# Jackz915/PackPPI

Measured on AMD Instinct MI355X. Metric: sampled residues/sec at 100 diffusion steps, higher is better.
Workload: dtype f32 (dense layers as split-f16: two f16 per operand, three f16 MFMAs per product, fp32 accumulate); 1 GPU; data/T1124_lig.pdb (L=739, 738 true residues), 1 complex per GPU; diffusion_steps=100, proximal=False, residues_per_gpu=738, residues_rank0=738, residues_total=738, mode=ode

## Files before the change

include/packppi_hip.h:

```cpp
#ifndef PACKPPI_HIP_H
#define PACKPPI_HIP_H

#include <stddef.h>
#include <stdint.h>

#ifdef __cplusplus
extern "C" {
#endif

typedef enum pp_status {
    PP_OK = 0,
    PP_ERR_INVALID = 1,
    PP_ERR_HIP = 2,
    PP_ERR_UNSUPPORTED = 3,
    PP_ERR_NO_DEVICE = 4
} pp_status;

typedef struct pp_plan pp_plan;
typedef struct pp_ctx pp_ctx;

#define PP_N_WEIGHTS 1439172u
#define PP_HIDDEN 128
#define PP_TOP_K 32
#define PP_MODE_ODE 0
// ... 216 lines not shown
#define PP_REFINE_MOVED 22
#define PP_REFINE_PCAP 16
#define PP_REFINE_MAX_SWEEPS 256
#define PP_REFINE_MAX_STEPS 16
#define PP_REFINE_MAX_BANDS 8
pp_status pp_chi_refine(pp_ctx *ctx, const float *chi0 , const uint8_t *fixed ,
                        const int8_t *place , const float *param ,
                        const float *ext , const float *radius ,
                        const uint8_t *acls , const uint8_t *aa_sep ,
                        const int32_t *link , const uint8_t *obst_polar , float delta,
                        int max_steps, int bands, float band, float cut, float hb_allow, float hb_weak, float hb_weak2, float hb_good2,
                        float reach, int max_sweeps, float *chi_out , int8_t *steps ,
                        float *xyz_out , float *hxyz_out ,
                        uint8_t *hmask_out , uint8_t *link_prev , int32_t *e ,
                        int32_t *trace , int32_t *sweeps ,
                        int32_t *converged , float *cand_xyz, float *cand_hxyz, uint8_t *cand_hmask,
                        int32_t *cand_mask, int32_t *energy , void *stream);

pp_status pp_time_kernel(pp_ctx *ctx, int which, int iters, float *avg_ms, void *stream);

pp_status pp_profile_kernel(pp_ctx *ctx, int which);
pp_status pp_profile_read(pp_ctx *ctx, float *total_ms, int *launches);

int pp_edge_variant(void);

int pp_has_range_check(void);
pp_status pp_range_check(unsigned long long *events, int reset);
pp_status pp_range_check_parts(unsigned long long *edge_events, unsigned long long *node_events, int reset);

pp_status pp_ctx_saturated(pp_ctx *ctx, int *flags, void *stream);

pp_status pp_ctx_live_rows(pp_ctx *ctx, int32_t *rows, int *count, void *stream);

#ifdef PP_DIAG
pp_status pp_debug_edge(pp_ctx *ctx, int layer, void *stream);
pp_status pp_debug_nm(pp_ctx *ctx, int layer, void *stream);
pp_status pp_debug_set_hE(pp_ctx *ctx, const float *src, size_t n);
pp_status pp_debug_buffer(pp_ctx *ctx, int which, float *dst, size_t n);
pp_status pp_debug_score_prefix(pp_ctx *ctx, const float *chi, float t, int n_launches, void *stream);
pp_status pp_debug_launch_plan(pp_ctx *ctx, int32_t out[5]);
void pp_debug_set_dbg(float *p);
void pp_debug_set_lds_pad(int bytes);
void pp_debug_set_edge_R(int R);
#endif

#ifdef __cplusplus
}
#endif
#endif
```

packppi_amd/csrc/pp_api.hip:

```cpp
#include <stdio.h>
#include <stdlib.h>

#include <algorithm>
#include <chrono>
#include <cmath>
#include <cstring>
#include <memory>
#include <new>
#include <string>
#include <vector>

#include "pp_internal.h"
#include "pp_pack.h"
#ifdef PP_EDGE_F16
#include "pp_rebalance.h"
#endif
#include "pp_topk_aten.h"

static thread_local std::string g_err;
void pp_set_error(const std::string &msg) { g_err = msg; }

extern "C" const char *pp_last_error(void) { return g_err.c_str(); }
extern "C" int pp_version(void) { return 101; }
#ifndef PP_BUILD_ID
// ... 45 lines not shown
                                 unsigned *__restrict__ sat) {
    const int i = blockIdx.x * blockDim.x + threadIdx.x;
    if (i >= rows * per_row) return;
    const int r = i / per_row, k = i - r * per_row;
    if (rmask && rmask[r] == 0.f) return;
    const float x = v[(size_t)r * row_stride + k];
    if (!(__builtin_fabsf(x) <= 3.402823466e38f)) atomicOr(sat, 4u);
}
static void flag_nonfinite(pp_ctx *c, const float *v, int row_stride, int per_row, hipStream_t s) {
    const int n = c->N * per_row;
    hipLaunchKernelGGL(k_flag_nonfinite, dim3((n + 255) / 256), dim3(256), 0, s, v, c->N, row_stride, per_row, c->b.residue_mask, c->sat);
}

extern "C" pp_status pp_ctx_saturated(pp_ctx *c, int *flags, void *stream) {
    if (!c || !flags) FAIL(PP_ERR_INVALID, "pp_ctx_saturated: null argument");
    hipStream_t s = static_cast<hipStream_t>(stream);
    unsigned v = 0;
    PP_HIP_CHECK(hipMemcpyAsync(&v, c->sat, sizeof(v), hipMemcpyDeviceToHost, s));
    PP_HIP_CHECK(hipStreamSynchronize(s));
    *flags = (int)v;
    return PP_OK;
}

extern "C" pp_status pp_ctx_live_rows(pp_ctx *c, int32_t *rows, int *count, void *stream) {
    if (!c || !rows || !count) FAIL(PP_ERR_INVALID, "pp_ctx_live_rows: null argument");
    if (!c->plan->has_network) FAIL(PP_ERR_INVALID, "pp_ctx_live_rows: plan was created without network weights");
    hipStream_t s = static_cast<hipStream_t>(stream);
    PP_HIP_CHECK(hipSetDevice(c->plan->device));
    int32_t cnt = 0;
    PP_HIP_CHECK(hipMemcpyAsync(rows, c->live_rows[0], (size_t)c->N * sizeof(int32_t), hipMemcpyDeviceToDevice, s));
    PP_HIP_CHECK(hipMemcpyAsync(&cnt, c->live_cnt[0], sizeof(cnt), hipMemcpyDeviceToHost, s));
    PP_HIP_CHECK(hipStreamSynchronize(s));
    *count = (int)cnt;
    return PP_OK;
}

static void side_chain_extents(const pp_tables *tables, float (&ext)[21]) {
    for (int S = 0; S < 21; S++) {
        float m = 0.f;
        for (int a = 4; a < 14; a++) {
            if (tables->atom14_mask[S * 14 + a] == 0.f) continue;
            const float *lp = tables->lit_positions + (S * 14 + a) * 3;
            float b = std::sqrt(lp[0] * lp[0] + lp[1] * lp[1] + lp[2] * lp[2]);
            const int g = tables->atom14_to_group[S * 14 + a];
            auto tlen = [&](int k) { const float *f = tables->default_frames + ((size_t)S * 8 + k) * 16; return std::sqrt(f[3] * f[3] + f[7] * f[7] + f[11] * f[11]); };
            if (g >= 4) for (int k = 4; k <= g; k++) b += tlen(k);
            else b += tlen(g);
            m = std::max(m, b);
        }
        ext[S] = m * 1.0001f + 1e-3f;
    }
}

struct PlanDeleter { void operator()(pp_plan *p) const { pp_plan_destroy(p); } };
struct CtxDeleter { void operator()(pp_ctx *c) const { pp_ctx_destroy(c); } };

extern "C" pp_status pp_plan_create(const float *weights, size_t n_weights, const pp_tables *tables, int device,
                                    pp_plan **out) {
    if (!tables || !out) FAIL(PP_ERR_INVALID, "pp_plan_create: null argument");
    WeightOff off = pp_weight_offsets();
    const bool has_net = weights != nullptr;
    if (has_net && (n_weights != off.total || off.total != PP_N_WEIGHTS))
        FAIL(PP_ERR_INVALID, "pp_plan_create: expected " + std::to_string(off.total) + " weights, got " +
                                 std::to_string(n_weights));
    if (has_net)
        for (size_t i = 0; i < n_weights; i++)
// ... 936 lines not shown
```

packppi_amd/csrc/pp_edge_f16.hip:

```cpp
#include "pp_internal.h"

PP_RANGE_COUNTER
PP_RANGE_READER(pp_edge_range_hits)

#include "pp_edge_tile.h"
typedef _Float16 h8 __attribute__((ext_vector_type(8)));

struct HT {
    h8 hi[2], lo[2];
};
typedef float f32x2v __attribute__((ext_vector_type(2)));
typedef _Float16 h2v __attribute__((ext_vector_type(2)));
typedef __fp16 fp16x2_t __attribute__((ext_vector_type(2)));
__device__ __forceinline__ h2v cvt2(f32x2v x) {
    const fp16x2_t r = __builtin_amdgcn_cvt_pkrtz(x[0], x[1]);
    return __builtin_bit_cast(h2v, r);
}
__device__ __forceinline__ f32x2v split_residual(h2v hh, f32x2v x) {
    const unsigned hp = __builtin_bit_cast(unsigned, hh);
    float d0, d1;
    asm("v_fma_mix_f32 %0, %1, -1.0, %2 op_sel_hi:[1,0,0]" : "=v"(d0) : "v"(hp), "v"(x[0]));
    asm("v_fma_mix_f32 %0, %1, -1.0, %2 op_sel:[1,0,0] op_sel_hi:[1,0,0]" : "=v"(d1) : "v"(hp), "v"(x[1]));
    return f32x2v{d0, d1};
}
// ... 51 lines not shown
    const float *frames;
    const float *pts;
    const float *PA, *PC;
    const float *hE_in;
    float *hE_out;
    float *S, *msum;
    const float *wstream;
    const float *params;
    const float *g3, *be3;
    const float *b_mid;
    const float *Z;
    const float *pts2, *PA2, *PC2, *b_mid2;
    float *Znm, *Zem;
    const float *ls_in, *ls_x1, *ls_out;
    unsigned *sat;
    float *dbg;
    int n_pairs;
    int mix_mode;
};
enum { P_BMID = 0, P_BOUT = 128, P_FOB = 256, P_G2 = 384, P_BE2 = 512, P_FIB = 640 };

#ifndef PP_WDEPTH
#define PP_WDEPTH 2
#endif
#ifndef PP_WDEPTH_R1
#define PP_WDEPTH_R1 2
#endif
#define WDEPTH_ (R == 1 ? PP_WDEPTH_R1 : PP_WDEPTH)
#if defined(PP_X_TS) && defined(PP_X_TS_FINE)
#define TSF(k) if constexpr ((k) >= PP_X_TS_FINE && (k) < PP_X_TS_FINE + 16) tsf[(k) - PP_X_TS_FINE] = (int)(__builtin_readcyclecounter() - ts0f);
#else
#define TSF(k)
#endif
#ifndef PP_WGS2
#define PP_WGS2 2
#endif
#ifndef PP_WGS
#define PP_WGS 3
#endif
#define NRING (WDEPTH_ + 1)
#ifdef PP_X_NOWLOAD
#define PP_X_NOWLOAD_ true
#else
#define PP_X_NOWLOAD_ false
#endif

#ifdef PP_X_E_NOMFMA
#define MFMA16(a, b, c) (c)
#else
#define MFMA16(a, b, c) __builtin_amdgcn_mfma_f32_32x32x16_f16((a), (b), (c), 0, 0, 0)
#endif

struct AOp {
    h8 r[4];
};
__device__ __forceinline__ void gload_A(const h8 *__restrict__ wq, int chunk, AOp &a) {
    int off = chunk * 1024;
    asm volatile("" : "+s"(off));
    const h8 *p = wq + off;
    a.r[0] = p[0]; a.r[1] = p[64]; a.r[2] = p[128]; a.r[3] = p[192];
}
template <int R, int T, bool SWAP>
__device__ __forceinline__ void mfma_x(const AOp &a, const HT (&x)[R][4], f32x16 (&acc)[R]) {
#pragma unroll
    for (int s = 0; s < 2; s++) {
        if (SWAP) {
#pragma unroll
            for (int r = 0; r < R; r++) acc[r] = MFMA16(x[r][T].hi[s], a.r[2 * s], acc[r]);
#pragma unroll
// ... 622 lines not shown
template <bool ST0, bool FUSE, bool LNS = false, bool WB = true, bool LIVE = false>
__global__ void __launch_bounds__(ET, 2)
k_edge_update_mix(EdgeArgs A) {
    extern __shared__ __attribute__((aligned(16))) float smem[];
    const int b = blockIdx.x;
    if constexpr (LIVE) {
        const int2 lrow = A.live_mix[b];
        if (lrow.x < 0) return;
        if (lrow.y >= 0) edge_update_body<2, ST0, FUSE, LNS, WB, true>(A, 0, smem, lrow);
        else edge_update_body<1, ST0, FUSE, LNS, WB, true>(A, 0, smem, lrow);
        return;
    }
    int pair = -1, single = -1;
    if (A.mix_mode == 2) {
        const int ns = gridDim.x - A.n_pairs;
        if (b < 2 * ns) { if (b & 1) single = b >> 1; else pair = b >> 1; }
        else pair = b - ns;
    } else if (A.mix_mode == 3) {
        const int ns = gridDim.x - A.n_pairs;
        if (b < ns) single = b; else pair = b - ns;
    } else {
        if (b < A.n_pairs) pair = b; else single = b - A.n_pairs;
    }
    if (pair >= 0) edge_update_body<2, ST0, FUSE, LNS, WB>(A, 2 * pair, smem);
    else edge_update_body<1, ST0, FUSE, LNS, WB>(A, 2 * A.n_pairs + single, smem);
}

template <bool ST0>
__global__ void __launch_bounds__(ET, 2)
k_node_message_mix(EdgeArgs A) {
    extern __shared__ __attribute__((aligned(16))) float smem[];
    const int b = blockIdx.x;
    const int ns = gridDim.x - A.n_pairs;
    if (b < ns) node_message_body<1, ST0>(A, 2 * A.n_pairs + b, smem);
    else node_message_body<2, ST0>(A, 2 * (b - ns), smem);
}

template <bool LNS>
__global__ void __launch_bounds__(ET, 1)
k_edge_static(EdgeArgs A) {
    extern __shared__ __attribute__((aligned(16))) float smem[];
    constexpr int R = 1;
    const int tid = threadIdx.x, lane = tid & 63;
    const int wave = __builtin_amdgcn_readfirstlane(tid >> 6);
    const int j = lane & 31, h = lane >> 5;
    const int n = blockIdx.x;
    const int K = A.K;
    if (A.rmask[n] == 0.f) return;
    constexpr int NCH = 8;
#if defined(PP_X_TS) && defined(PP_X_TS_FINE)
    const unsigned long long ts0f = __builtin_readcyclecounter();
    int tsf[16] = {0};
#endif
    PROLOGUE_PIPE(NCH)
    HT x[1][4];
    f32x16 acc[1];
    const int jj = j < K ? j : K - 1;
    const float *hrow = A.hE_in + ((size_t)n * K + jj) * 128;
#pragma unroll
    for (int t = 0; t < 4; t++) {
        load_tile(hrow + 32 * t, h, acc[0]);
        if constexpr (LNS) scale_tile(A.ls_in + 32 * t, h, acc[0], acc[0]);
        unsigned nosat = 0;
        split_tile<false>(acc[0], x[0][t], nosat);
    }
#pragma unroll
    for (int r = 0; r < 16; r++) acc[0][r] = 0.f;
    WSTAGE(0, NCH, acc, (mfma_x<1, 0, false>(AK, x, acc)))
// ... 255 lines not shown
        for (int lns = 0; lns < 2 && ok; lns++) ok = set(reinterpret_cast<const void *>(mix_kernel(false, lns, false, true)), MAX_SMEM);
        for (int st0 = 0; st0 < 2 && ok; st0++)
            for (int lns = 0; lns < 2 && ok; lns++)
                ok = set(reinterpret_cast<const void *>(mix_kernel(st0, lns, true)), MAX_SMEM) &&
                     set(reinterpret_cast<const void *>(mix_kernel(st0, lns, false)), MAX_SMEM);
        ok = ok && set(reinterpret_cast<const void *>(k_node_message_mix<true>), MAX_SMEM) &&
             set(reinterpret_cast<const void *>(k_node_message_mix<false>), MAX_SMEM);
        int dev = 0;
        hipDeviceProp_t prop;
        if (hipGetDevice(&dev) == hipSuccess && hipGetDeviceProperties(&prop, dev) == hipSuccess)
            g_num_cu = prop.multiProcessorCount;
        if (g_num_cu <= 0) g_num_cu = 256;
    }
    return ok;
}

static int g_forced_R = -1;
#ifdef PP_DIAG
extern "C" void pp_debug_set_edge_R(int R) { g_forced_R = R; }
#endif
static int pick_R(int N) {
    if (g_forced_R < 0) {
        const char *e = PP_GETENV("PP_EDGE_R");
        g_forced_R = e ? atoi(e) : 0;
    }
    if (g_forced_R >= 1 && g_forced_R <= PP_RMAX) return g_forced_R;
    return N > PP_WGS * g_num_cu ? 2 : 1;
}

static int g_mix = -1;
static bool use_mix(int N) {
    if (g_mix < 0) {
        const char *e = PP_GETENV("PP_EDGE_MIX");
        g_mix = e ? atoi(e) : 3;
    }
    if (g_forced_R >= 1 || !g_mix) return false;
    return N > 2 * g_num_cu && N <= 3 * g_num_cu;
}
static int mix_pairs(int N) { return (N + 2) / 3; }

void pp_edge_occupancy(int *node_msg, int *edge_upd) {
    edge_attrs();
    (void)hipOccupancyMaxActiveBlocksPerMultiprocessor(node_msg, reinterpret_cast<const void *>(nm_kernel_r(1, false)), ET, nm_smem(1));
    (void)hipOccupancyMaxActiveBlocksPerMultiprocessor(edge_upd, reinterpret_cast<const void *>(eu_kernel_r(1, false)), ET, eu_smem(1));
}

#define EDGE_ATTR_CHECK()                                                                                   \
    if (!edge_attrs()) {                                                                                    \
        pp_set_error("hipFuncSetAttribute(MaxDynamicSharedMemorySize) failed for the edge kernels");        \
        return PP_ERR_HIP;                                                                                  \
    }

pp_status pp_launch_edge_static(pp_ctx *c, hipStream_t s) {
    EDGE_ATTR_CHECK()
    EdgeArgs A = edge_args(c, 0, false);
    A.wstream = c->plan->static_stream;
    if (c->plan->ln_scale) hipLaunchKernelGGL(k_edge_static<true>, dim3(c->N), dim3(ET), ST_SMEM, s, A);
    else hipLaunchKernelGGL(k_edge_static<false>, dim3(c->N), dim3(ET), ST_SMEM, s, A);
    PP_HIP_CHECK(hipGetLastError());
    return PP_OK;
}

pp_status pp_launch_node_message(pp_ctx *c, int layer, hipStream_t s) {
    EDGE_ATTR_CHECK()
    EdgeArgs A = edge_args(c, layer, false);
    static const char *nm_env = PP_GETENV("PP_NM_R");
    static const int nm_R = nm_env ? atoi(nm_env) : 0;
    const int R = (nm_R >= 1 && nm_R <= PP_RMAX) ? nm_R : pick_R(c->N);
    static const char *nmix_env = PP_GETENV("PP_NM_MIX");
    static const bool nmix = !(nmix_env && atoi(nmix_env) == 0);
    if (nmix && !(nm_R >= 1 && nm_R <= PP_RMAX) && use_mix(c->N)) {
        A.n_pairs = mix_pairs(c->N);
        const int singles = c->N - 2 * A.n_pairs > 0 ? c->N - 2 * A.n_pairs : 0;
        PP_LAUNCH(c, (layer == 0 ? k_node_message_mix<true> : k_node_message_mix<false>), dim3(A.n_pairs + singles), dim3(ET),
                  nm_smem(2), s, A);
        PP_HIP_CHECK(hipGetLastError());
        return PP_OK;
    }
    PP_LAUNCH(c, nm_kernel_r(R, layer == 0), dim3((c->N + R - 1) / R), dim3(ET), nm_smem(R), s, A);
    PP_HIP_CHECK(hipGetLastError());
    return PP_OK;
}

#ifdef PP_DIAG
pp_status pp_edge_launch_plan(int N, int *R, int *mixed, int *n_pairs) {
    EDGE_ATTR_CHECK()
    *mixed = use_mix(N) ? 1 : 0;
    *R = pick_R(N);
    *n_pairs = *mixed ? mix_pairs(N) : 0;
    return PP_OK;
}
#endif

extern "C" int pp_edge_variant(void) { return 1; }
bool pp_edge_fused() { return PP_FUSED; }

pp_status pp_launch_edge_update(pp_ctx *c, int layer, bool keep_hE, hipStream_t s, const PPLive *live) {
    EDGE_ATTR_CHECK()
    if (layer < 0 || layer > 1) { pp_set_error("pp_launch_edge_update: layer must be 0 or 1"); return PP_ERR_INVALID; }
    if (live && (layer != 1 || keep_hE || !PP_FUSED)) { pp_set_error("pp_launch_edge_update: the live-row launch is layer 1's, without write-back"); return PP_ERR_INVALID; }
    EdgeArgs A = edge_args(c, layer, true);
    const int R = pick_R(c->N);
    const bool mixed = use_mix(c->N);
    if (live) {
        if (mixed && !live->mix) { pp_set_error("pp_launch_edge_update: the mixed launch has no live-row work table for this context"); return PP_ERR_INVALID; }
        if (mixed) A.live_mix = live->mix;
        else A.live_rows = live->rows;
    }
    const bool lns = c->plan->ln_scale != nullptr;
    if (lns && !PP_FUSED) { pp_set_error("pp_launch_edge_update: a plan with LayerNorm operand scales needs the fused build"); return PP_ERR_UNSUPPORTED; }
    if (mixed) {
        A.n_pairs = mix_pairs(c->N);
        A.mix_mode = g_mix;
        const int singles = c->N - 2 * A.n_pairs > 0 ? c->N - 2 * A.n_pairs : 0;
        const int wgs = live ? (c->N < 2 * g_num_cu ? c->N : 2 * g_num_cu) : A.n_pairs + singles;
        PP_LAUNCH(c, mix_kernel(layer == 0, lns, keep_hE, live != nullptr), dim3(wgs), dim3(ET), eu_smem(2) > eu_smem(1) ? eu_smem(2) : eu_smem(1), s, A);
        PP_HIP_CHECK(hipGetLastError());
        return PP_OK;
    }
    PP_LAUNCH(c, eu_kernel_r(R, layer == 0, lns, keep_hE, live != nullptr), dim3((c->N + R - 1) / R), dim3(ET), eu_smem(R), s, A);
    PP_HIP_CHECK(hipGetLastError());
    return PP_OK;
}
```

packppi_amd/csrc/pp_internal.h:

```cpp
#pragma once
#include <hip/hip_runtime.h>
#include <hip/hip_ext.h>
#include <cmath>
#include <vector>
#include <mutex>
#include <stdint.h>
#include <string>

#include "../../include/packppi_hip.h"

#if defined(PP_LAB) && !defined(PP_DIAG)
#define PP_DIAG
#endif
#if !defined(PP_LAB) &&                                                                                                       \
    (defined(PP_X_TS) || defined(PP_X_TS_FINE) || defined(PP_X_NOWLOAD) || defined(PP_X_E_NOMFMA) || defined(PP_X_NOSAT) ||      \
     defined(PP_WDEPTH) || defined(PP_WDEPTH_R1) || defined(PP_NXB_R1) || defined(PP_WGS2) || defined(PP_WGS) ||                 \
     defined(PP_NM_WGS2) ||                                                                                                  \
     defined(PP_LDS_PAD) || defined(PP_NO_FUSE_NM) || defined(PP_NU_DEPTH))
#error "PP_X_* / tuning switches compile laboratory variants (most give wrong results): add -DPP_LAB and build a TAGGED library (python -m packppi_amd.build --tag NAME -DPP_LAB -DPP_X_...)"
#endif
#ifdef PP_DIAG
#define PP_GETENV(name) getenv(name)
#else
#define PP_GETENV(name) ((const char *)nullptr)
// ... 266 lines not shown
    const float sgn = (sg > 0.f) ? 1.f : ((sg < 0.f) ? -1.f : 0.f);
    const float ang = sgn * acosf(pp_dot_t(n1, n2));
    return (ang != ang) ? 0.f : ang;
}
#endif

struct pp_affinity {
    int device;
    bool network;
    float *buf;
    const float *mut_bias, *seq_emb;
    const float *f0T, *f0_b, *f2T, *f2_b;
    const float *d0T, *d0_b, *d2T, *d2_b, *d4_w, *d4_b;
};

struct PPRng {
    const pp_rng_row *tab;
    uint32_t seed_lo, seed_hi;
};

struct PPPin {
    const uint8_t *fixed;
    const float *chi_ref;
    float *traj;
    float sigma;
    int renoise;
};

struct PPLive {
    const int32_t *rows;
    const int2 *mix;
};

pp_status pp_launch_live_rows(pp_ctx *c, int set, const uint8_t *fixed, hipStream_t s);
pp_status pp_launch_rng_table(pp_ctx *c, bool keys_set, hipStream_t s);
pp_status pp_launch_noise_seeded(pp_ctx *c, uint64_t seed, int step, float *noise, uint32_t *words, hipStream_t s);
pp_status pp_launch_add_noise_seeded(pp_ctx *c, const float *chi0, float sigma, uint64_t seed, float *chi, hipStream_t s);
pp_status pp_launch_affinity_embed(pp_ctx *c, const pp_affinity *a, const int64_t *rtype, const float *sc_sincos,
                                   const int64_t *mut_mask, const float *hV_pret, hipStream_t s);
pp_status pp_launch_prepare(pp_ctx *c, hipStream_t s, const int64_t *E_idx = nullptr);
pp_status pp_launch_node_embed(pp_ctx *c, const float *chi, const StepParams &sp, hipStream_t s);
pp_status pp_launch_node_embed_rows(pp_ctx *c, const float *chi, const float *t_rows, hipStream_t s);
struct NodeEval {
    float *chi;
    int step, mode;
    const float *noise;
    const StepParams *cur;
    const StepParams *next;
    const PPRng *rng;
    const PPPin *pin;
};
pp_status pp_launch_node_update(pp_ctx *c, int layer, int last_mode, const NodeEval &ev, hipStream_t s);
pp_status pp_launch_edge_static(pp_ctx *c, hipStream_t s);
#ifdef PP_EDGE_F16
pp_status pp_launch_edge_embed_f16(pp_ctx *c, hipStream_t s);
#endif
pp_status pp_launch_node_message(pp_ctx *c, int layer, hipStream_t s);
bool pp_edge_fused();
pp_status pp_launch_edge_update(pp_ctx *c, int layer, bool keep_hE, hipStream_t s, const PPLive *live = nullptr);
pp_status pp_launch_atom14(pp_ctx *c, const float *chi, float *xyz, hipStream_t s);
pp_status pp_launch_clash(pp_ctx *c, const float *xyz, float *per_res, float *dchi, hipStream_t s, bool use_candidates = false);
pp_status pp_launch_proximal(pp_ctx *c, const float *chi, float lamda, int nsteps, float *traj,
                             float *chi_last, float *losses, hipStream_t s);
pp_status pp_launch_proximal_packed(pp_ctx *c, const float *chi, float lamda, int nsteps, bool norm_given, float *traj,
                                    float *chi_last, float *chi_accepted, float *losses, hipStream_t s,
                                    const uint8_t *fixed = nullptr, uint8_t *moved = nullptr);
// ... 18 lines not shown
```

packppi_amd/csrc/pp_prepare.hip:

```cpp
#include "pp_internal.h"
#include "pp_topk_aten.h"

#define KNN_THREADS 256
#define KNN_PAR_MAX 2047

#pragma clang fp contract(off)

__device__ __forceinline__ float dist_eps(const float *a, const float *b, float eps) {
    float dx = a[0] - b[0], dy = a[1] - b[1], dz = a[2] - b[2];
    float s = dx * dx;
    s = s + dy * dy;
    s = s + dz * dz;
    return sqrtf(s + eps);
}

__global__ void k_frames(const float *__restrict__ X, int N, float *__restrict__ frames,
                         float *__restrict__ bbpos) {
    int n = blockIdx.x * blockDim.x + threadIdx.x;
    if (n >= N) return;
    const float *x = X + (size_t)n * 42;
    float Nn[3], CA[3], C[3], O[3];
    for (int k = 0; k < 3; k++) { Nn[k] = x[k]; CA[k] = x[3 + k]; C[k] = x[6 + k]; O[k] = x[9 + k]; }
    float a[3], b[3];
    for (int k = 0; k < 3; k++) { a[k] = C[k] - CA[k]; b[k] = Nn[k] - CA[k]; }
// ... 300 lines not shown

pp_status pp_launch_prepare(pp_ctx *c, hipStream_t s, const int64_t *E_idx) {
    const int N = c->N;
    if (E_idx) {
        PP_HIP_CHECK(hipMemsetAsync(c->scal, 0, sizeof(int), s));
        hipLaunchKernelGGL(k_import_graph, dim3((N * 32 + 255) / 256), dim3(256), 0, s, E_idx, c->seg, c->b.residue_mask, N, c->K,
                           c->eidx, c->mask_att, reinterpret_cast<int *>(c->scal));
    } else {
    hipLaunchKernelGGL(k_frames, dim3((N + 127) / 128), dim3(128), 0, s, c->b.X, N, c->frames, c->bbpos);
    const size_t smem = (size_t)c->L * sizeof(pp_tk_pair) + 2 * (KNN_PAR_MAX + 1) * sizeof(short);
    if (smem > 64 * 1024) {
        PP_HIP_CHECK(hipFuncSetAttribute(reinterpret_cast<const void *>(k_knn),
                                         hipFuncAttributeMaxDynamicSharedMemorySize, (int)smem));
    }
    hipLaunchKernelGGL(k_knn, dim3(N), dim3(KNN_THREADS), smem, s, c->b.X, c->b.residue_mask, c->seg, c->K,
                       c->plan->knn_ties, c->L, c->eidx, c->mask_att);
    }
#ifdef PP_EDGE_F16
    return pp_launch_edge_embed_f16(c, s);
#else
    const pp_plan *p = c->plan;
    size_t smem2 = (size_t)32 * EF_STRIDE * sizeof(float);
    hipLaunchKernelGGL(k_edge_embed, dim3(N), dim3(EF_THREADS), smem2, s, c->bbpos, c->eidx, c->b.residue_index,
                       c->b.chain_indices, c->K, p->edge_emb_T, p->w + p->off.edge_emb_b,
                       p->w + p->off.norm_edges_g, p->w + p->off.norm_edges_b, c->hE0);
    PP_HIP_CHECK(hipGetLastError());
    return PP_OK;
#endif
}

#define LIVE_THREADS 1024
__global__ void __launch_bounds__(LIVE_THREADS)
k_live_rows(const float *__restrict__ rmask, const float *__restrict__ scm, const uint8_t *__restrict__ fixed, int N,
            int32_t *__restrict__ rows, int2 *__restrict__ mix, int32_t *__restrict__ cnt) {
    __shared__ int part[LIVE_THREADS];
    const int t = threadIdx.x;
    const int per = (N + LIVE_THREADS - 1) / LIVE_THREADS;
    const int lo = min(t * per, N), hi = min(lo + per, N);
    auto is_live = [&](int i) {
        const float *m = scm + (size_t)i * 4;
        return rmask[i] != 0.f && (m[0] != 0.f || m[1] != 0.f || m[2] != 0.f || m[3] != 0.f) && !(fixed && fixed[i] != 0);
    };
    int c = 0;
    for (int i = lo; i < hi; i++) c += is_live(i) ? 1 : 0;
    part[t] = c;
    __syncthreads();
    for (int d = 1; d < LIVE_THREADS; d <<= 1) {
        const int v = t >= d ? part[t - d] : 0;
        __syncthreads();
        part[t] += v;
        __syncthreads();
    }
    const int M = part[LIVE_THREADS - 1];
    int o = part[t] - c;
    for (int i = lo; i < hi; i++)
        if (is_live(i)) rows[o++] = i;
    for (int i = M + t; i < N + 2; i += LIVE_THREADS) rows[i] = -1;
    if (mix) {
        const int np = (M + 2) / 3, ns = max(M - 2 * np, 0);
        __syncthreads();
        for (int b = t; b < N; b += LIVE_THREADS) {
            int2 e = make_int2(-1, -1);
            if (b < np) e = make_int2(rows[2 * b], rows[2 * b + 1]);
            else if (b - np < ns) e.x = rows[2 * np + b - np];
            mix[b] = e;
        }
    }
    if (t == 0) cnt[0] = M;
}

pp_status pp_launch_live_rows(pp_ctx *c, int set, const uint8_t *fixed, hipStream_t s) {
    const int num_cu = c->plan->num_cu;
    const bool want_mix = c->N > 2 * num_cu && c->N <= 3 * num_cu;
    hipLaunchKernelGGL(k_live_rows, dim3(1), dim3(LIVE_THREADS), 0, s, c->b.residue_mask, c->b.SC_D_mask, fixed, c->N,
                       c->live_rows[set], want_mix ? c->live_mix[set] : nullptr, c->live_cnt[set]);
    c->live_mix_set[set] = want_mix;
    PP_HIP_CHECK(hipGetLastError());
    return PP_OK;
}
```

packppi_amd/lib.py:

```python
import ctypes as C
import os

import numpy as np
import torch

from . import constants as rc
from .weights import check_state_dict

_LIB_PATH = os.environ.get("PACKPPI_LIB") or os.path.join(os.path.dirname(os.path.abspath(__file__)), "csrc", "libpackppi_hip.so")
_lib = None

SYMBOLS = ("pp_version", "pp_last_error", "pp_build_id", "pp_plan_set_knn_ties", "pp_plan_set_annealed_temp", "pp_plan_rebalanced_chains", "pp_rebalance_weights_host", "pp_plan_ln_scaled_features", "pp_ln_operand_scales_host", "pp_topk_aten_host", "pp_plan_create", "pp_plan_destroy", "pp_plan_set_clash_params",
           "pp_complex_prepare", "pp_complex_prepare_packed", "pp_ctx_destroy", "pp_ctx_get_graph", "pp_ctx_set_graph", "pp_score", "pp_sample", "pp_atom14",
           "pp_clash", "pp_proximal", "pp_proximal_packed", "pp_time_kernel", "pp_profile_kernel", "pp_profile_read", "pp_edge_variant", "pp_has_range_check", "pp_range_check", "pp_range_check_parts", "pp_ctx_saturated",
           "pp_affinity_create", "pp_affinity_destroy", "pp_affinity_encode", "pp_affinity_predict",
           "pp_score_rows", "pp_so2_set_grids", "pp_so2_score", "pp_dsm_loss",
           "pp_ctx_set_rng_keys", "pp_noise_seeded", "pp_add_noise_seeded", "pp_sample_seeded",
           "pp_sample_partial", "pp_proximal_pinned", "pp_ctx_live_rows", "pp_ensemble_reduce", "pp_ctx_shell",
           "pp_ensemble_recombine", "pp_ctx_set_obstacles", "pp_sasa", "pp_sample_guided", "pp_sample_corrected",
           "pp_disulfide_close", "pp_polar", "pp_hydrogens", "pp_clashscore", "pp_hnet_optimize", "pp_chi_refine")


FIX_MODES = {"hold": 0, "renoise": 1}
KNN_TIES = {"lower_index": 0, "aten_cpu": 1, "aten_member": 2}
SELECT = {None: 0, "none": 0, "clash": 1, "medoid": 2}
SHELL_MODES = {"ca": 0, "atom": 1}
SHELL_OTHER_CHAIN = 1


class EnsembleResult(dict):

    def __getattr__(self, k):
        try:
            return self[k]
        except KeyError as e:
            raise AttributeError(k) from e


DISULFIDE_OVERFLOW = ("disulfides: more cysteine pairs lie within cb_max than the candidate list of this context holds "
                      "(min(N (N - 1) / 2, 64 N)); nothing was bonded -- lower cb_max or name the pairs")


class DisulfideResult(EnsembleResult):

    def bonds(self):
        if bool((self["count"] < 0).any()):
            raise RuntimeError(DISULFIDE_OVERFLOW)
        p = self["partner"].reshape(-1).tolist()
        return [(a, b) for a, b in enumerate(p) if b > a]


# ... 58 lines not shown
    lib.pp_ctx_set_graph.argtypes = [vp, vp, vp]
    lib.pp_score.argtypes = [vp, vp, f, vp, vp, vp]
    lib.pp_sample.argtypes = [vp, vp, vp, i, i, vp, vp]
    lib.pp_atom14.argtypes = [vp, vp, vp, vp]
    lib.pp_clash.argtypes = [vp, vp, vp, vp, vp]
    lib.pp_proximal.argtypes = [vp, vp, f, i, vp, vp, vp, vp]
    lib.pp_proximal_packed.argtypes = [vp, vp, f, i, vp, vp, vp, vp, vp, vp]
    lib.pp_time_kernel.argtypes = [vp, i, i, C.POINTER(C.c_float), vp]
    lib.pp_profile_kernel.argtypes = [vp, i]
    lib.pp_profile_read.argtypes = [vp, C.POINTER(C.c_float), C.POINTER(C.c_int)]
    lib.pp_edge_variant.argtypes = []
    lib.pp_has_range_check.argtypes = []
    lib.pp_has_range_check.restype = C.c_int
    lib.pp_range_check.argtypes = [C.POINTER(C.c_ulonglong), i]
    lib.pp_range_check_parts.argtypes = [C.POINTER(C.c_ulonglong), C.POINTER(C.c_ulonglong), i]
    lib.pp_ctx_saturated.argtypes = [vp, C.POINTER(C.c_int), vp]
    lib.pp_edge_variant.restype = C.c_int
    lib.pp_affinity_create.argtypes = [vp, C.c_size_t, i, C.POINTER(vp)]
    lib.pp_affinity_destroy.argtypes = [vp]
    lib.pp_affinity_destroy.restype = None
    lib.pp_affinity_encode.argtypes = [vp, vp, vp, vp, vp, vp, vp, vp]
    lib.pp_affinity_predict.argtypes = [vp, vp, vp, vp, i, i, vp, vp, vp]
    lib.pp_score_rows.argtypes = [vp, vp, vp, vp, vp, vp]
    lib.pp_so2_set_grids.argtypes = [vp, vp, i]
    lib.pp_so2_score.argtypes = [vp, vp, C.c_size_t, i, vp, vp, i, vp]
    lib.pp_dsm_loss.argtypes = [vp, vp, vp, vp, vp, vp, vp, vp]
    lib.pp_ctx_set_rng_keys.argtypes = [vp, vp, vp]
    lib.pp_noise_seeded.argtypes = [vp, C.c_uint64, i, vp, vp, vp]
    lib.pp_add_noise_seeded.argtypes = [vp, vp, f, C.c_uint64, vp, vp]
    lib.pp_sample_seeded.argtypes = [vp, vp, vp, i, i, C.c_uint64, vp]
    lib.pp_sample_partial.argtypes = [vp, vp, vp, vp, i, vp, i, i, C.c_uint64, vp, vp]
    lib.pp_proximal_pinned.argtypes = [vp, vp, vp, f, i, vp, vp, vp, vp, vp, vp, vp]
    lib.pp_ctx_live_rows.argtypes = [vp, vp, C.POINTER(C.c_int), vp]
    lib.pp_ensemble_reduce.argtypes = [vp, vp, i, vp, i, vp, vp, vp, vp, vp, vp, vp]
    lib.pp_ctx_shell.argtypes = [vp, vp, i, f, i, vp, vp, vp, vp]
    lib.pp_ensemble_recombine.argtypes = [vp, vp, i, vp, i, vp, vp, vp, vp, vp, vp, vp]
    lib.pp_ctx_set_obstacles.argtypes = [vp, vp, vp, i, vp]
    lib.pp_sasa.argtypes = [vp, vp, vp, vp, i, f, vp, vp, vp, vp]
    lib.pp_disulfide_close.argtypes = [vp, vp, vp, vp, i, f, f, f, vp, vp, vp, vp, vp]
    lib.pp_polar.argtypes = [vp, vp, vp, vp, vp, f, f, vp, vp, vp, vp, vp]
    lib.pp_hydrogens.argtypes = [vp, vp, vp, vp, vp, vp, vp, vp, vp]
    lib.pp_clashscore.argtypes = [vp, vp, vp, vp, vp, vp, vp, vp, vp, vp, f, f, vp, vp, vp, vp, vp]
    lib.pp_hnet_optimize.argtypes = [vp] * 20 + [f] * 6 + [C.c_int] + [vp] * 13
    lib.pp_chi_refine.argtypes = [vp] * 11 + [f, i, i] + [f] * 7 + [i] + [vp] * 16
    lib.pp_sample_guided.argtypes = [vp, vp, vp, vp, i, vp, i, i, C.c_uint64, vp, f, vp, vp, vp]
    lib.pp_sample_corrected.argtypes = [vp, vp, vp, vp, i, vp, i, i, C.c_uint64, vp, vp, f, vp, vp, vp, vp]
    _lib = lib
    return lib


def _check(status, what):
    if status != 0:
        msg = load().pp_last_error()
        raise RuntimeError(f"{what} failed (pp_status {status}): {msg.decode() if msg else ''}")


def _stream(device):
    return C.c_void_p(torch.cuda.current_stream(device).cuda_stream)


def _ptr(t):
    return C.c_void_p(t.data_ptr()) if t is not None else C.c_void_p(0)


def _host_f32(seq):
    return np.ascontiguousarray(torch.as_tensor(seq, dtype=torch.float32).cpu().numpy())
# ... 922 lines not shown
            cx, ch = self._new(R, 9, self.B, self.L, 14, 3), self._new(R, 9, self.B, self.L, rc.PP_H_MAX, 3)
            cm = self._new(R, 9, self.B, self.L, rc.PP_H_MAX, dtype=torch.uint8)
            ck, en = self._new(R, self.B, self.L, dtype=torch.int32), self._new(R, self.B, self.L, 9, dtype=torch.int32)
            cc = self._new(R, self.B, self.L, 4)
        at = lambda t, r: _ptr(t[r]) if t is not None else None
        for r, delta in enumerate(deltas):
            out = self._new(self.B, self.L, 4)
            if cc is not None:
                cc[r].copy_(cur)
            _check(load().pp_chi_refine(
                self.handle, _ptr(cur), _ptr(fx), _ptr(tabs.place), _ptr(tabs.param), _ptr(self._rf_ext), _ptr(radius), _ptr(tabs.acls),
                _ptr(tabs.aa_sep), _ptr(link), _ptr(op), delta, int(max_steps), int(bands), float(band), float(cut), float(hb_allow),
                float(hb_weak), float(f32(hb_weak) * f32(hb_weak)), float(f32(hb_good) * f32(hb_good)), float(reach), ms, _ptr(out),
                _ptr(steps[r]), _ptr(xyz), _ptr(hxyz), _ptr(hmask), _ptr(link_prev), _ptr(e_round[r]), _ptr(trace[r]), _ptr(sweeps[r]),
                _ptr(converged[r]), at(cx, r), at(ch, r), at(cm, r), at(ck, r), at(en, r), self._stream()), "pp_chi_refine")
            cur = out
        rotation = sum(steps[r].float() * deltas[r] for r in range(R))
        return EnsembleResult(chi=cur, chi0=chi_in, xyz=xyz, hxyz=hxyz, hmask=hmask, link_prev=link_prev, steps=steps,
                              moved=(steps != 0).any(-1).any(0), rotation=rotation, e=torch.stack([e_round[0, ..., 0], e_round[-1, ..., 1]], -1),
                              e_round=e_round, F=torch.stack([trace[0, :, 0], trace[-1, :, -1]], -1).to(torch.int64), trace=trace,
                              sweeps=sweeps, converged=converged, deltas=deltas, radius=radius, fixed=fx, cand_xyz=cx, cand_hxyz=ch,
                              cand_hmask=cm, cand_mask=ck, cand_chi=cc, energy=en)

    def saturated(self) -> int:
        v = C.c_int(0)
        _check(load().pp_ctx_saturated(self.handle, C.byref(v), self._stream()), "pp_ctx_saturated")
        return int(v.value)

    def live_rows(self):
        rows, n = self._new(self.n_rows, dtype=torch.int32), C.c_int(0)
        _check(load().pp_ctx_live_rows(self.handle, _ptr(rows), C.byref(n), self._stream()), "pp_ctx_live_rows")
        return rows[:int(n.value)]

    def time_kernel(self, which: int, iters: int = 20) -> float:
        ms = C.c_float(0.0)
        _check(load().pp_time_kernel(self.handle, int(which), int(iters), C.byref(ms), self._stream()),
               "pp_time_kernel")
        return float(ms.value)

    def profile_kernel(self, which: int):
        _check(load().pp_profile_kernel(self.handle, int(which)), "pp_profile_kernel")

    def profile_read(self):
        ms, n = C.c_float(0.0), C.c_int(0)
        _check(load().pp_profile_read(self.handle, C.byref(ms), C.byref(n)), "pp_profile_read")
        return (float(ms.value) / max(n.value, 1), int(n.value))

    def __del__(self):
        h = getattr(self, "handle", None)
        if h and _lib is not None:
            _lib.pp_ctx_destroy(h)
            self.handle = None


SO2_GRID = 5001
_so2_grids_on = set()


def so2_grids():
    X_MIN, X_N, SIGMA_MIN, SIGMA_MAX, SIGMA_N = 1e-5, 5000, 3e-3, 2, 5000
    xs, ss = [], []
    for PI in (1 / 2 * np.pi, np.pi):
        xs.append(10 ** np.linspace(np.log10(X_MIN), 0, X_N + 1) * PI)
        ss.append(10 ** np.linspace(np.log10(SIGMA_MIN), np.log10(SIGMA_MAX), SIGMA_N + 1) * PI)
    return np.ascontiguousarray(np.stack(xs)), np.ascontiguousarray(np.stack(ss))

# ... 74 lines not shown
```

Baseline: 65120 residues/s.

## Generalize pair/single row mixing to occupancy-slot shape and switch default mix mode

Measured after the change: 65850 residues/s (median of 6 runs). 1.1% higher.

```diff
diff --git a/include/packppi_hip.h b/include/packppi_hip.h
--- a/include/packppi_hip.h
+++ b/include/packppi_hip.h
@@ -272,6 +272,9 @@
 
 pp_status pp_ctx_live_rows(pp_ctx *ctx, int32_t *rows, int *count, void *stream);
 
+pp_status pp_ctx_live_mix(pp_ctx *ctx, int32_t *mix, int *workgroups);
+pp_status pp_live_mix_host(const int32_t *rows, int M, int N, int num_cu, int32_t *mix, int *workgroups);
+
 #ifdef PP_DIAG
 pp_status pp_debug_edge(pp_ctx *ctx, int layer, void *stream);
 pp_status pp_debug_nm(pp_ctx *ctx, int layer, void *stream);
diff --git a/packppi_amd/csrc/pp_api.hip b/packppi_amd/csrc/pp_api.hip
--- a/packppi_amd/csrc/pp_api.hip
+++ b/packppi_amd/csrc/pp_api.hip
@@ -101,6 +101,30 @@
     PP_HIP_CHECK(hipMemcpyAsync(&cnt, c->live_cnt[0], sizeof(cnt), hipMemcpyDeviceToHost, s));
     PP_HIP_CHECK(hipStreamSynchronize(s));
     *count = (int)cnt;
+    return PP_OK;
+}
+
+extern "C" pp_status pp_ctx_live_mix(pp_ctx *c, int32_t *mix, int *workgroups) {
+    if (!c || !mix || !workgroups) FAIL(PP_ERR_INVALID, "pp_ctx_live_mix: null argument");
+    if (!c->plan->has_network) FAIL(PP_ERR_INVALID, "pp_ctx_live_mix: plan was created without network weights");
+    PP_HIP_CHECK(hipSetDevice(c->plan->device));
+    *workgroups = 0;
+    if (!c->live_mix_set[0]) return PP_OK;
+    PP_HIP_CHECK(hipDeviceSynchronize());
+    PP_HIP_CHECK(hipMemcpy(mix, c->live_mix[0], (size_t)c->N * sizeof(int2), hipMemcpyDeviceToHost));
+    *workgroups = pp_live_mix_grid(c->N, c->plan->num_cu, PP_WGS2);
+    return PP_OK;
+}
+
+extern "C" pp_status pp_live_mix_host(const int32_t *rows, int M, int N, int num_cu, int32_t *mix, int *workgroups) {
+    if (!rows || !mix || !workgroups || M < 0 || M > N || num_cu < 1) FAIL(PP_ERR_INVALID, "pp_live_mix_host: null argument, M outside 0 .. N or no compute unit");
+    const PPEdgeShape sh = pp_edge_shape(M, num_cu, PP_WGS2);
+    for (int b = 0; b < N; b++) {
+        const int2 e = pp_live_mix_entry(rows, sh, b);
+        mix[2 * b] = e.x;
+        mix[2 * b + 1] = e.y;
+    }
+    *workgroups = pp_live_mix_size(N, num_cu, PP_WGS2) ? pp_live_mix_grid(N, num_cu, PP_WGS2) : 0;
     return PP_OK;
 }
 
diff --git a/packppi_amd/csrc/pp_edge_f16.hip b/packppi_amd/csrc/pp_edge_f16.hip
--- a/packppi_amd/csrc/pp_edge_f16.hip
+++ b/packppi_amd/csrc/pp_edge_f16.hip
@@ -107,9 +107,6 @@
 #else
 #define TSF(k)
 #endif
-#ifndef PP_WGS2
-#define PP_WGS2 2
-#endif
 #ifndef PP_WGS
 #define PP_WGS 3
 #endif
@@ -798,8 +795,13 @@
     extern __shared__ __attribute__((aligned(16))) float smem[];
     const int b = blockIdx.x;
     const int ns = gridDim.x - A.n_pairs;
-    if (b < ns) node_message_body<1, ST0>(A, 2 * A.n_pairs + b, smem);
-    else node_message_body<2, ST0>(A, 2 * (b - ns), smem);
+    if (A.mix_mode == 3) {
+        if (b < ns) node_message_body<1, ST0>(A, 2 * A.n_pairs + b, smem);
+        else node_message_body<2, ST0>(A, 2 * (b - ns), smem);
+    } else {
+        if (b < A.n_pairs) node_message_body<2, ST0>(A, 2 * b, smem);
+        else node_message_body<1, ST0>(A, 2 * A.n_pairs + (b - A.n_pairs), smem);
+    }
 }
 
 template <bool LNS>
@@ -1121,12 +1123,16 @@
 static bool use_mix(int N) {
     if (g_mix < 0) {
         const char *e = PP_GETENV("PP_EDGE_MIX");
-        g_mix = e ? atoi(e) : 3;
+        g_mix = e ? atoi(e) : 1;
     }
     if (g_forced_R >= 1 || !g_mix) return false;
     return N > 2 * g_num_cu && N <= 3 * g_num_cu;
 }
-static int mix_pairs(int N) { return (N + 2) / 3; }
+static int mix_pairs(int N) { return pp_edge_shape(N, g_num_cu, PP_WGS2).pairs; }
+static bool use_live_mix(int N) {
+    (void)use_mix(N);
+    return g_forced_R < 1 && g_mix && pp_live_mix_size(N, g_num_cu, PP_WGS2);
+}
 
 void pp_edge_occupancy(int *node_msg, int *edge_upd) {
     edge_attrs();
@@ -1160,6 +1166,7 @@
     static const bool nmix = !(nmix_env && atoi(nmix_env) == 0);
     if (nmix && !(nm_R >= 1 && nm_R <= PP_RMAX) && use_mix(c->N)) {
         A.n_pairs = mix_pairs(c->N);
+        A.mix_mode = g_mix;
         const int singles = c->N - 2 * A.n_pairs > 0 ? c->N - 2 * A.n_pairs : 0;
         PP_LAUNCH(c, (layer == 0 ? k_node_message_mix<true> : k_node_message_mix<false>), dim3(A.n_pairs + singles), dim3(ET),
                   nm_smem(2), s, A);
@@ -1190,7 +1197,7 @@
     if (live && (layer != 1 || keep_hE || !PP_FUSED)) { pp_set_error("pp_launch_edge_update: the live-row launch is layer 1's, without write-back"); return PP_ERR_INVALID; }
     EdgeArgs A = edge_args(c, layer, true);
     const int R = pick_R(c->N);
-    const bool mixed = use_mix(c->N);
+    const bool mixed = live ? use_live_mix(c->N) : use_mix(c->N);
     if (live) {
         if (mixed && !live->mix) { pp_set_error("pp_launch_edge_update: the mixed launch has no live-row work table for this context"); return PP_ERR_INVALID; }
         if (mixed) A.live_mix = live->mix;
@@ -1199,10 +1206,10 @@
     const bool lns = c->plan->ln_scale != nullptr;
     if (lns && !PP_FUSED) { pp_set_error("pp_launch_edge_update: a plan with LayerNorm operand scales needs the fused build"); return PP_ERR_UNSUPPORTED; }
     if (mixed) {
-        A.n_pairs = mix_pairs(c->N);
+        A.n_pairs = live ? 0 : mix_pairs(c->N);
         A.mix_mode = g_mix;
         const int singles = c->N - 2 * A.n_pairs > 0 ? c->N - 2 * A.n_pairs : 0;
-        const int wgs = live ? (c->N < 2 * g_num_cu ? c->N : 2 * g_num_cu) : A.n_pairs + singles;
+        const int wgs = live ? pp_live_mix_grid(c->N, g_num_cu, PP_WGS2) : A.n_pairs + singles;
         PP_LAUNCH(c, mix_kernel(layer == 0, lns, keep_hE, live != nullptr), dim3(wgs), dim3(ET), eu_smem(2) > eu_smem(1) ? eu_smem(2) : eu_smem(1), s, A);
         PP_HIP_CHECK(hipGetLastError());
         return PP_OK;
diff --git a/packppi_amd/csrc/pp_internal.h b/packppi_amd/csrc/pp_internal.h
--- a/packppi_amd/csrc/pp_internal.h
+++ b/packppi_amd/csrc/pp_internal.h
@@ -322,6 +322,38 @@
     const int2 *mix;
 };
 
+#ifndef PP_WGS2
+#define PP_WGS2 2
+#endif
+struct PPEdgeShape {
+    int pairs, one_row;
+    bool pairs_first;
+};
+__host__ __device__ inline PPEdgeShape pp_edge_shape(int M, int num_cu, int slots) {
+    const int S = slots * num_cu;
+    PPEdgeShape sh = {(M + 1) / 2, 0, true};
+    if (M <= S) sh.pairs = 0;
+    else if (2 * M <= 3 * S) sh.pairs = (M + 2) / 3;
+    else if (M > 2 * S && M <= 3 * S) sh.pairs = S;
+    sh.one_row = M > 2 * sh.pairs ? M - 2 * sh.pairs : 0;
+    return sh;
+}
+__host__ __device__ inline int2 pp_live_mix_entry(const int32_t *rows, const PPEdgeShape &sh, int b) {
+    int2 e = make_int2(-1, -1);
+    const int p = sh.pairs_first ? b : b - sh.one_row, q = sh.pairs_first ? b - sh.pairs : b;
+    if (p >= 0 && p < sh.pairs) e = make_int2(rows[2 * p], rows[2 * p + 1]);
+    else if (q >= 0 && q < sh.one_row) e.x = rows[2 * sh.pairs + q];
+    return e;
+}
+inline bool pp_live_mix_size(int N, int num_cu, int slots) {
+    const int S = slots * num_cu;
+    return (N > S && 2 * N <= 3 * S) || (N > 2 * S && N <= 3 * S);
+}
+inline int pp_live_mix_grid(int N, int num_cu, int slots) {
+    const int S = slots * num_cu;
+    return N > 2 * S ? N - S : S;
+}
+
 pp_status pp_launch_live_rows(pp_ctx *c, int set, const uint8_t *fixed, hipStream_t s);
 pp_status pp_launch_rng_table(pp_ctx *c, bool keys_set, hipStream_t s);
 pp_status pp_launch_noise_seeded(pp_ctx *c, uint64_t seed, int step, float *noise, uint32_t *words, hipStream_t s);
diff --git a/packppi_amd/csrc/pp_prepare.hip b/packppi_amd/csrc/pp_prepare.hip
--- a/packppi_amd/csrc/pp_prepare.hip
+++ b/packppi_amd/csrc/pp_prepare.hip
@@ -356,7 +356,7 @@
 #define LIVE_THREADS 1024
 __global__ void __launch_bounds__(LIVE_THREADS)
 k_live_rows(const float *__restrict__ rmask, const float *__restrict__ scm, const uint8_t *__restrict__ fixed, int N,
-            int32_t *__restrict__ rows, int2 *__restrict__ mix, int32_t *__restrict__ cnt) {
+            int32_t *__restrict__ rows, int2 *__restrict__ mix, int32_t *__restrict__ cnt, int num_cu, int slots) {
     __shared__ int part[LIVE_THREADS];
     const int t = threadIdx.x;
     const int per = (N + LIVE_THREADS - 1) / LIVE_THREADS;
@@ -381,23 +381,18 @@
         if (is_live(i)) rows[o++] = i;
     for (int i = M + t; i < N + 2; i += LIVE_THREADS) rows[i] = -1;
     if (mix) {
-        const int np = (M + 2) / 3, ns = max(M - 2 * np, 0);
+        const PPEdgeShape sh = pp_edge_shape(M, num_cu, slots);
         __syncthreads();
-        for (int b = t; b < N; b += LIVE_THREADS) {
-            int2 e = make_int2(-1, -1);
-            if (b < np) e = make_int2(rows[2 * b], rows[2 * b + 1]);
-            else if (b - np < ns) e.x = rows[2 * np + b - np];
-            mix[b] = e;
-        }
+        for (int b = t; b < N; b += LIVE_THREADS) mix[b] = pp_live_mix_entry(rows, sh, b);
     }
     if (t == 0) cnt[0] = M;
 }
 
 pp_status pp_launch_live_rows(pp_ctx *c, int set, const uint8_t *fixed, hipStream_t s) {
     const int num_cu = c->plan->num_cu;
-    const bool want_mix = c->N > 2 * num_cu && c->N <= 3 * num_cu;
+    const bool want_mix = pp_live_mix_size(c->N, num_cu, PP_WGS2);
     hipLaunchKernelGGL(k_live_rows, dim3(1), dim3(LIVE_THREADS), 0, s, c->b.residue_mask, c->b.SC_D_mask, fixed, c->N,
-                       c->live_rows[set], want_mix ? c->live_mix[set] : nullptr, c->live_cnt[set]);
+                       c->live_rows[set], want_mix ? c->live_mix[set] : nullptr, c->live_cnt[set], num_cu, PP_WGS2);
     c->live_mix_set[set] = want_mix;
     PP_HIP_CHECK(hipGetLastError());
     return PP_OK;
diff --git a/packppi_amd/lib.py b/packppi_amd/lib.py
--- a/packppi_amd/lib.py
+++ b/packppi_amd/lib.py
@@ -16,7 +16,7 @@
            "pp_affinity_create", "pp_affinity_destroy", "pp_affinity_encode", "pp_affinity_predict",
            "pp_score_rows", "pp_so2_set_grids", "pp_so2_score", "pp_dsm_loss",
            "pp_ctx_set_rng_keys", "pp_noise_seeded", "pp_add_noise_seeded", "pp_sample_seeded",
-           "pp_sample_partial", "pp_proximal_pinned", "pp_ctx_live_rows", "pp_ensemble_reduce", "pp_ctx_shell",
+           "pp_sample_partial", "pp_proximal_pinned", "pp_ctx_live_rows", "pp_ctx_live_mix", "pp_live_mix_host", "pp_ensemble_reduce", "pp_ctx_shell",
            "pp_ensemble_recombine", "pp_ctx_set_obstacles", "pp_sasa", "pp_sample_guided", "pp_sample_corrected",
            "pp_disulfide_close", "pp_polar", "pp_hydrogens", "pp_clashscore", "pp_hnet_optimize", "pp_chi_refine")
 
@@ -141,6 +141,8 @@
     lib.pp_sample_partial.argtypes = [vp, vp, vp, vp, i, vp, i, i, C.c_uint64, vp, vp]
     lib.pp_proximal_pinned.argtypes = [vp, vp, vp, f, i, vp, vp, vp, vp, vp, vp, vp]
     lib.pp_ctx_live_rows.argtypes = [vp, vp, C.POINTER(C.c_int), vp]
+    lib.pp_ctx_live_mix.argtypes = [vp, vp, C.POINTER(C.c_int)]
+    lib.pp_live_mix_host.argtypes = [vp, i, i, i, vp, C.POINTER(C.c_int)]
     lib.pp_ensemble_reduce.argtypes = [vp, vp, i, vp, i, vp, vp, vp, vp, vp, vp, vp]
     lib.pp_ctx_shell.argtypes = [vp, vp, i, f, i, vp, vp, vp, vp]
     lib.pp_ensemble_recombine.argtypes = [vp, vp, i, vp, i, vp, vp, vp, vp, vp, vp, vp]
@@ -1129,6 +1131,11 @@
         _check(load().pp_ctx_live_rows(self.handle, _ptr(rows), C.byref(n), self._stream()), "pp_ctx_live_rows")
         return rows[:int(n.value)]
 
+    def live_mix(self):
+        mix, n = torch.empty(self.n_rows, 2, dtype=torch.int32), C.c_int(0)
+        _check(load().pp_ctx_live_mix(self.handle, _ptr(mix), C.byref(n)), "pp_ctx_live_mix")
+        return (mix, int(n.value)) if n.value else (None, 0)
+
     def time_kernel(self, which: int, iters: int = 20) -> float:
         ms = C.c_float(0.0)
         _check(load().pp_time_kernel(self.handle, int(which), int(iters), C.byref(ms), self._stream()),
```
